# Penguin77jp/RaytracingMin

Hardware: AMD Instinct MI355X
Metric: Msamples/s (W*H*spp/s), Cornell box 1080p@1024spp (higher is better)
Workload: dtype f64; 1 GPU; cornellBoxSetting.json rows 0:1080 of 1920x1080 1024spp (SS 4 x S 64), L1 repaired, max_bounces 8, seed 0x5EED, host-libm sin/cos (RTM_MODE_HOST_TRIG), interleaved 8-row bands over 1 GPU(s) + one gather; sample_split_waves_per_tile=8, collective=none (one rank, frame stays in HBM)

## Files before the change

### raytracingmin_amd/csrc/rtm_kernels.hip

```cpp
#include <hip/hip_runtime.h>

#include <cfloat>
#include <cmath>
#include <cstdio>
#include <cstdlib>
#include <cstring>
#include <algorithm>
#include <atomic>
#include <thread>
#include <map>
#include <memory>
#include <mutex>
#include <shared_mutex>
#include <tuple>
#include <string>
#include <type_traits>
#include <vector>

#include "../../include/rtm.h"
#include "rtm_device.h"
#include "rtm_host.h"
#include "rtm_path.h"
#include "rtm_scene_facts.h"

// ... 709 lines not shown
    }
    return false;
}

template <class M, int UNROLL, typename RecT, int WPE, unsigned F>
static void launch_render_depth(const RenderParams& P, unsigned grid, hipStream_t stream) {
    const size_t pad = debug_lds_pad();
    if constexpr ((F & kPack8) != 0 && sizeof(RecT) == 1) {
        if (P.max_bounces >= 0 && P.max_bounces <= 8 && P.scene.n < 256) {
            if constexpr ((F & kDefer) != 0 && UNROLL == -8) {
                if (launch_exact_n<M, F, RecT, 16, WPE>(P, grid, stream)) return;
            }
            launch_tiles<M, F, UNROLL, RecT, 16, WPE>(P, grid, pad, stream);
            return;
        }
    }
    if constexpr ((F & kDefer) != 0 && sizeof(RecT) == 1) {
        if (P.scene.n < 256) {
            constexpr unsigned FL = (F & ~(kPack8 | kSteal)) | kPackL;
            if constexpr (UNROLL == -8) {
                if (launch_exact_n<M, FL, RecT, 0, WPE>(P, grid, stream)) return;
            }
            launch_tiles<M, FL, UNROLL, RecT, 0, WPE>(P, grid, pad, stream);
            return;
        }
    }
    constexpr unsigned FR = F & (kLdsTab | kPark | kStamp);
    if (!needs_pool(P)) launch_tiles<M, FR, UNROLL, RecT, 16, WPE>(P, grid, pad, stream);
    else launch_tiles<M, FR, UNROLL, RecT, deep_lds_levels<RecT>(), WPE>(P, grid, pad, stream);
}

template <int UNROLL, unsigned F>
static void launch_fold(const RenderParams& P, unsigned grid, hipStream_t stream) {
    if (P.split > 1) {
        launch_render_depth<MathFast, UNROLL, uint8_t, 4, F | kSplit>(P, P.split_first + P.n_tiles * P.split, stream);
        launch_split_finalize(P, stream);
    } else {
        launch_render_depth<MathFast, UNROLL, uint8_t, 4, F>(P, grid, stream);
    }
    if constexpr ((F & kSteal) != 0) launch_steal_finalize(P, grid, stream);
}
template <unsigned F>
static void launch_fold_lds(const RenderParams& P, unsigned grid, hipStream_t stream) {
    if (P.scene.n < 8) launch_fold<-8, F>(P, grid, stream);
    else launch_fold<8, F>(P, grid, stream);
}

static void launch_render(int variant, const RenderParams& P, unsigned grid, hipStream_t stream) {
    const int n = P.scene.n;
    constexpr unsigned kFold = kPark | kPack8 | kDefer;
    if (variant == kVariantFastLds && n > kLdsTableMaxSpheres) variant = kVariantFastGlobal;
    switch (variant) {
        case kVariantRef:
            if (n <= 256) launch_render_depth<MathRef, 1, uint8_t, 1, 0>(P, grid, stream);
            else launch_render_depth<MathRef, 1, uint32_t, 1, 0>(P, grid, stream);
            return;
        case kVariantFastLds:
            if (P.scene.plane != nullptr) launch_fold<8, kLdsTab | kFold | kPlanes>(P, grid, stream);
            else if (P.steal_ws != nullptr) launch_fold_lds<kLdsTab | kFold | kSteal>(P, grid, stream);
            else launch_fold_lds<kLdsTab | kFold>(P, grid, stream);
            return;
        case kVariantGlobalDefer:
            launch_fold<8, kFold>(P, grid, stream);
            return;
        case kVariantFp32: {
            const size_t lds = (((size_t)n * kFp32Row * sizeof(float) + 15) & ~(size_t)15) + 10 * sizeof(double);
            render_fp32_kernel<<<grid, 64, lds, stream>>>(P);
            return;
        }
        case kVariantPrimaryReuse:
            if (n < 8) launch_tiles<MathFast, kLdsTab | kFold | kReuse, -8, uint8_t, 16, 4>(P, grid, debug_lds_pad(), stream);
            else launch_tiles<MathFast, kLdsTab | kFold | kReuse, 8, uint8_t, 16, 4>(P, grid, debug_lds_pad(), stream);
            return;
// ... 1544 lines not shown
```

### raytracingmin_amd/csrc/rtm_kernels_tol.hip

```cpp
#define RTM_NS rtm_tol
#define RTM_TOL 1
#include <hip/hip_runtime.h>

#include <cmath>
#include <cstdlib>
#include <cstring>
#include <map>
#include <mutex>
#include <vector>

#include "rtm_internal.h"
#include "rtm_render_kernel.h"

namespace rtm_tol {

static bool compact_launch(const RenderParams& P) {
    const double cam = std::sqrt(P.cam_org.x * P.cam_org.x + P.cam_org.y * P.cam_org.y + P.cam_org.z * P.cam_org.z);
    return (P.scene.fold_flags & kSceneCompact) != 0u && cam <= kCompactExtent;
}
static bool expanded_form_launch(const RenderParams& P) {
    const unsigned e = (P.scene.fold_flags >> kSceneAxisReachShift) & kSceneAxisReachMask;
    const double cam = std::sqrt(P.cam_org.x * P.cam_org.x + P.cam_org.y * P.cam_org.y + P.cam_org.z * P.cam_org.z);
    return e != 0u && cam <= std::ldexp(1.0, (int)e - 128);
}
// ... 14 lines not shown
#define RTM_AXIS_CASE(k, sig)                                                                                    \
    if (P.scene.n == k && P.scene.axis_pat == ((sig) & 0xFFFFu) && ((shared_k << kAxisSharedKShift) | pairs) == ((sig) & ~0xFFFFu) && axis) { \
        launch_tiles<MathFast, F, axis_unroll(k, sig), uint8_t, LDS_D, kTolWavesPerSimd>(P, grid, lds_pad, stream); \
        return;                                                                                                  \
    }
    if constexpr (kPairsShape) {
        RTM_AXIS_CASE(7, kAxisSigCornell7Pairs)
    }
    RTM_AXIS_CASE(7, kAxisSigCornell7Walls)
#undef RTM_AXIS_CASE
#define RTM_AXIS_CASE(k, sig)                                                                                    \
    if (P.scene.n == k && P.scene.axis_pat == sig && axis) {                                                     \
        launch_tiles<MathFast, F, axis_unroll(k, sig), uint8_t, LDS_D, kTolWavesPerSimd>(P, grid, lds_pad, stream); \
        return;                                                                                                  \
    }
    if constexpr ((F & kPackL) != 0) {
        RTM_AXIS_CASE(7, kAxisSigCornell7)
    } else {
        RTM_AXIS_SIGNATURES(RTM_AXIS_CASE)
        switch (P.scene.n) {
            case 3: launch_tiles<MathFast, F, -103, uint8_t, LDS_D, kTolWavesPerSimd>(P, grid, lds_pad, stream); return;
            case 5: launch_tiles<MathFast, F, -105, uint8_t, LDS_D, kTolWavesPerSimd>(P, grid, lds_pad, stream); return;
            case 7: launch_tiles<MathFast, F, -107, uint8_t, LDS_D, kTolWavesPerSimd>(P, grid, lds_pad, stream); return;
            default: break;
        }
    }
#undef RTM_AXIS_CASE
    if (P.scene.n < 8) launch_tiles<MathFast, F, -8, uint8_t, LDS_D, kTolWavesPerSimd>(P, grid, lds_pad, stream);
    else launch_tiles<MathFast, F, 8, uint8_t, LDS_D, kTolWavesPerSimd>(P, grid, lds_pad, stream);
}

template <unsigned F>
static void launch_row(const RenderParams& P, unsigned grid, size_t lds_pad, hipStream_t stream) {
    if (P.split > 1) {
        launch_n<F | kSplit>(P, P.split_first + P.n_tiles * P.split, lds_pad, stream);
        launch_split_finalize(P, stream);
    } else {
        launch_n<F>(P, grid, lds_pad, stream);
    }
    if constexpr ((F & kSteal) != 0) launch_steal_finalize(P, grid, stream);
}

__global__ void tol_math_probe_kernel(int op, const double* __restrict__ a, const double* __restrict__ b, size_t n,
                                      double* __restrict__ out, const double2* __restrict__ tab) {
    const size_t i = (size_t)blockIdx.x * blockDim.x + threadIdx.x;
    if (i >= n) return;
    if (op >= 52 && op <= 54) {
        const size_t j = i & ~(size_t)7;
        double bb = 0.0, D4 = 0.0;
        if (b && j + 7 < n) {
            const D3 org = d3(a[j], a[j + 1], a[j + 2]), dir = d3(a[j + 3], a[j + 4], a[j + 5]);
            const unsigned pat = (unsigned)b[j];
            const double c = b[j + 1];
            if (pat >= 1u && pat <= 3u) {
                if (op == 52) {
                    const double4 g = double4{pat == 1u ? c : 0.0, pat == 2u ? c : 0.0, pat == 3u ? c : 0.0, b[j + 2]};
                    sphere_disc_ref(g, pat, org, dir, AxisSharedRef(org, dir), bb, D4);
                } else {
                    const AxisShared A(org, dir);
                    sphere_disc(double4{}, AxisRow{c, b[j + 3], b[j + 4]}, pat, op == 54, A.oo + b[j + 4], org, dir, A, bb, D4);
                }
            }
        }
        out[i] = (i & 7) == 0 ? bb : (i & 7) == 1 ? D4 : 0.0;
        return;
    }
    if (op == 55 || op == 56 || op == 61 || op == 62) {
        const size_t j = i & ~(size_t)7;
        double dis = DBL_MAX;
        int hit = -1;
        bool fell_back = false, general = false, again = false;
        if (b && n >= 56 && j + 7 < n) {
            const D3 org = d3(a[j], a[j + 1], a[j + 2]), dir = d3(a[j + 3], a[j + 4], a[j + 5]);
            SceneGlobal sc{};
            sc.v.geom = reinterpret_cast<const double4*>(b);
            sc.v.n = 7;
            if (op == 55) sphere_chunk<MathFast, 7, SceneGlobal, false, kAxisSigCornell7Pairs>(sc, 0, org, dir, dis, hit, &fell_back);
            else if (op == 61) sphere_chunk<MathFast, 7, SceneGlobal, false, kAxisSigCornell7Pairs>(sc, 0, org, dir, dis, hit, &fell_back, &general, &again);
            else if (op == 62) sphere_chunk<MathFast, 7, SceneGlobal, false, kAxisSigCornell7Pairs, true>(sc, 0, org, dir, dis, hit, &fell_back, &general, &again);
            else sphere_chunk<MathFast, 7, SceneGlobal, false, kAxisSigCornell7Walls>(sc, 0, org, dir, dis, hit);
        }
        const bool f2 = op >= 61 ? general : fell_back, f3 = op >= 61 && fell_back;
        const unsigned s = (unsigned)(i & 7);
        out[i] = s == 0u ? dis : s == 1u ? (double)hit : s == 2u ? (f2 ? 1.0 : 0.0) : s == 3u ? (f3 ? 1.0 : 0.0) : s == 4u ? (again ? 1.0 : 0.0) : 0.0;
        return;
    }
    if (op == 57 || op == 58) {
        if (i * 8 + 7 >= n) return;
        const double* q = a + i * 8;
        const RngPixelKey pk{(uint32_t)q[0], (uint32_t)q[1]};
        RngStream st{(uint32_t)q[2], (uint32_t)q[3]};
        const uint32_t n_next = (uint32_t)q[4];
        const bool ended = q[5] != 0.0;
        uint32_t w[4] = {0u, 0u, 0u, 0u};
        (void)rng_next_mi(st);
        if (op == 57) {
            const RngStream m = rng_merged_mix(ended, pk, n_next, st);
            if (ended) {
                w[2] = m.ctr;
                w[3] = m.k1;
            } else {
                w[0] = rng_bits_to_mi(m.ctr);
                w[1] = (uint32_t)(rng_bits_to_u01(m.k1) * 16777216.0);
                w[2] = st.ctr + 2u * 0x9E3779B9u;
                w[3] = st.k1;
            }
        } else if (ended) {
            st = rng_open(pk, n_next);
            w[2] = st.ctr;
            w[3] = st.k1;
        } else {
            w[0] = rng_next_mi(st);
            w[1] = (uint32_t)(rng_next(st) * 16777216.0);
            w[2] = st.ctr;
            w[3] = st.k1;
        }
// ... 183 lines not shown
```

### raytracingmin_amd/csrc/rtm_render_kernel.h

```cpp
#pragma once
#include <type_traits>

#include "rtm_path.h"

namespace RTM_NS {

struct RenderParams {
    SceneView scene;
    int W, H, S, SS;
    int row_begin, row_end;
    int band_count, band_index;
    int tiles_x;
    int mode, max_bounces;
    unsigned total_samples;
    unsigned sample_begin, sample_end, seeded;
    double preview_scale;
    float rate;
    double dSS, dS;
    double inv_ss, inv_s;
    D3 cam_org, ax, by, cz;
    uint64_t seed_mult;
    double* __restrict__ out64;
    float* __restrict__ out32;
    uint8_t* __restrict__ out8;
// ... 1014 lines not shown
        }
    }

    if constexpr (PARK) acc = d3(park[0 * 64 + lane], park[1 * 64 + lane], park[2 * 64 + lane]);
    if (STEAL && whole) {
    } else if (whole) {
        int px, py;
        pixel_xy(px, py);
        store_pixel(P, (px < P.W) && (py < P.row_end), px, py, acc);
    } else if (n_first == P.sample_begin) {
        unsigned hf, split_tile;
        split_wave(hf, split_tile);
        double* dst = P.partial + (size_t)split_tile * 192 + lane;
        dst[0] = acc.x;
        dst[64] = acc.y;
        dst[128] = acc.z;
    }
    if (P.counters) {
        if constexpr (DEFER) {
            if (lane == 0) {
                atomicAdd(P.counters + 0, (unsigned long long)w_casts);
                atomicAdd(P.counters + 1, (unsigned long long)w_bounces);
                atomicAdd(P.counters + 2, (unsigned long long)w_draws);
            }
        } else {
            wave_add_counter(P.counters + 0, pc.casts);
            wave_add_counter(P.counters + 1, pc.bounces);
            wave_add_counter(P.counters + 2, pc.draws);
        }
        if (stack.overflow) atomicOr(P.counters + 3, 1ull);
    }
}

__global__ __launch_bounds__(256) void split_finalize_kernel(const RenderParams P) {
    extern __shared__ __attribute__((aligned(16))) unsigned char lds_raw[];
    double* slot = reinterpret_cast<double*>(lds_raw);
    unsigned* present = reinterpret_cast<unsigned*>(slot + (size_t)P.split_len * 64u * 3u);
    const int tid = threadIdx.x, lane = tid & 63, chan = tid >> 6;
    const unsigned tile = frame_tile(P, P.split_first + blockIdx.x);
    if (tile == ~0u) return;
    const int tx = tile % P.tiles_x, ty = tile / P.tiles_x;
    const int px = tx * 8 + (lane & 7), py = band_row(P, ty, lane >> 3);
    const bool valid = (px < P.W) && (py < P.row_end);
    const unsigned plane_sz = P.split_len * 64u;
    double acc = chan < 3 ? P.partial[(size_t)blockIdx.x * 192 + chan * 64 + lane] : 0.0;
    for (unsigned f = 1; f < P.split; ++f) {
        const unsigned char* rows = P.contrib + ((size_t)blockIdx.x * (P.split - 1u) + (f - 1u)) * P.split_len * kTermRowBytes;
        unsigned n_terms = P.split_counts[(size_t)blockIdx.x * (P.split - 1u) + (f - 1u)];
        n_terms = n_terms <= plane_sz ? n_terms : 0u;
        for (unsigned m = (unsigned)tid; m < P.split_len * 2u; m += 256u) present[m] = 0u;
        __syncthreads();
        for (unsigned e = (unsigned)tid; e < n_terms; e += 256u) {
            const unsigned char* row = rows + (size_t)(e >> 6) * kTermRowBytes;
            const double* v = reinterpret_cast<const double*>(row) + (e & 63u);
            const unsigned tag = reinterpret_cast<const unsigned short*>(row + 3 * 64 * sizeof(double))[e & 63u];
            if ((tag >> 6) >= P.split_len) continue;
            const unsigned at = (tag >> 6) * 64u + (tag & 63u);
            slot[at] = v[0];
            slot[plane_sz + at] = v[64];
            slot[2 * plane_sz + at] = v[128];
            atomicOr(&present[(tag >> 6) * 2u + ((tag >> 5) & 1u)], 1u << (tag & 31u));
        }
        __syncthreads();
        if (chan < 3) {
            const double* mine = slot + (size_t)chan * plane_sz + lane;
            const unsigned* bits = present + (lane >> 5);
            for (unsigned m = 0; m < P.split_len; ++m)
                if ((bits[m * 2u] >> (lane & 31)) & 1u) acc = acc + mine[m * 64u];
        }
        __syncthreads();
    }
    if (chan < 3) slot[chan * 64 + lane] = acc;
    __syncthreads();
    if (chan == 0) store_pixel(P, valid, px, py, d3(slot[lane], slot[64 + lane], slot[128 + lane]));
}

__global__ __launch_bounds__(64) void steal_finalize_kernel(const RenderParams P) {
    extern __shared__ __attribute__((aligned(16))) unsigned char lds_raw[];
    unsigned short* idx = reinterpret_cast<unsigned short*>(lds_raw);
    const int lane = threadIdx.x;
    const unsigned tile = blockIdx.x;
    const unsigned ftile = frame_tile(P, tile);
    if (ftile == ~0u) return;
    const int tx = ftile % P.tiles_x, ty = ftile / P.tiles_x;
    const int px = tx * 8 + (lane & 7), py = band_row(P, ty, lane >> 3);
    const bool valid = (px < P.W) && (py < P.row_end);
    const unsigned char* blk = P.steal_ws + (size_t)tile * steal_tile_bytes(P.steal_rows);
    unsigned n_terms = reinterpret_cast<const unsigned*>(blk)[0];
    unsigned end_own = reinterpret_cast<const unsigned short*>(blk + 128)[lane];
    n_terms = n_terms <= P.steal_rows * 64u ? n_terms : 0u;
    const unsigned floor_chk = P.sample_end > P.steal_depth ? P.sample_end - P.steal_depth : 0u;
    end_own = (n_terms != 0u && end_own >= floor_chk && end_own <= P.sample_end) ? end_own : P.sample_end;
    const double* part = reinterpret_cast<const double*>(blk + kStealHdrBytes) + lane;
    D3 acc = d3(part[0], part[64], part[128]);
    if (n_terms != 0u) {
        const unsigned total = P.sample_end;
        const unsigned floor_s = total > P.steal_depth ? total - P.steal_depth : 0u;
        const unsigned char* rows = blk + kStealHdrBytes + 3 * 64 * sizeof(double);
        for (unsigned k = (unsigned)lane; k < P.steal_depth * 32u; k += 64u) reinterpret_cast<unsigned*>(idx)[k] = 0xFFFFFFFFu;
        __syncthreads();
        for (unsigned e = (unsigned)lane; e < n_terms; e += 64u) {
            const unsigned tag = reinterpret_cast<const unsigned*>(rows + (size_t)(e >> 6) * kStealRowBytes + 3 * 64 * sizeof(double))[e & 63u];
            const unsigned ts = tag & 0xFFFFu, tv = (tag >> 16) & 63u;
            if (ts >= floor_s && ts < total) idx[(ts - floor_s) * 64u + tv] = (unsigned short)e;
        }
        __syncthreads();
        if (valid) {
            for (unsigned s = end_own; s < total; ++s) {
                const unsigned e = idx[(s - floor_s) * 64u + (unsigned)lane];
                if (e >= n_terms) continue;
                const double* v = reinterpret_cast<const double*>(rows + (size_t)(e >> 6) * kStealRowBytes) + (e & 63u);
                acc = acc + d3(v[0], v[64], v[128]);
            }
        }
    }
    store_pixel(P, valid, px, py, acc);
}

template <class M, unsigned F, int UNROLL, typename RecT, int LDS_D, int WPE>
void launch_tiles(RenderParams P, unsigned grid, size_t pad, hipStream_t stream) {
    const size_t lds = render_lds_bytes<F, RecT, LDS_D>(P.scene.n, lds_rows_for(UNROLL), pad, &P.unit_tab);
    render_tiles_kernel<M, F, UNROLL, RecT, LDS_D, WPE><<<grid, 64, lds, stream>>>(P);
}
inline void launch_split_finalize(const RenderParams& P, hipStream_t stream) {
    split_finalize_kernel<<<P.n_tiles, 256, (size_t)P.split_len * (64 * 3 * sizeof(double) + 2 * sizeof(unsigned)), stream>>>(P);
}
inline void launch_steal_finalize(const RenderParams& P, unsigned grid, hipStream_t stream) {
    const unsigned n_whole = P.split > 1 ? P.split_first : grid;
    if (n_whole) steal_finalize_kernel<<<n_whole, 64, (size_t)P.steal_depth * 64 * sizeof(unsigned short), stream>>>(P);
}

__global__ __launch_bounds__(64) void prim_prepass_kernel(const RenderParams P, unsigned long long* __restrict__ masks,
                                                          double* __restrict__ dirs) {
    const int lane = threadIdx.x;
    const unsigned tile = blockIdx.x;
    const unsigned ftile = frame_tile(P, tile);
    if (ftile == ~0u) return;
    auto store_dir = [&](const unsigned sub, const D3 d) {
        const unsigned all_s = (unsigned)(P.SS * P.SS);
        double* q = dirs + ((size_t)tile * all_s + sub) * 192 + (unsigned)lane;
        constexpr int kStep = 64;
        __builtin_nontemporal_store(d.x, q);
        __builtin_nontemporal_store(d.y, q + kStep);
        __builtin_nontemporal_store(d.z, q + 2 * kStep);
    };
    const int x = (int)(ftile % (unsigned)P.tiles_x) * 8 + (lane & 7);
    const int y = band_row(P, (int)(ftile / (unsigned)P.tiles_x), lane >> 3);
    const double cam[9] = {P.ax.x, P.ax.y, P.ax.z, P.by.x, P.by.y, P.by.z, P.cz.x, P.cz.y, P.cz.z};
    [[maybe_unused]] unsigned long long mask = 0ull;
    const unsigned all = (unsigned)(P.SS * P.SS);
    const unsigned sub_end = (P.sample_end - 1u) / (unsigned)P.S + 2u;
    for (unsigned sub = P.sample_begin / (unsigned)P.S; sub < (sub_end < all ? sub_end : all); ++sub) {
        if (dirs == nullptr && (masks == nullptr || sub >= 64u)) break;
        const D3 d = primary_dir_lds(P, cam, x, y, (int)(sub / (unsigned)P.SS) + 1, (int)(sub % (unsigned)P.SS) + 1);
#if RTM_TOL
        if (masks != nullptr && sub < 64u) {
            SceneGlobal sc;
            sc.v = P.scene;
            mask |= primary_tie_risk(sc, P.cam_org, d) ? (1ull << sub) : 0ull;
        }
#endif
        if (dirs != nullptr) store_dir(sub, d);
// ... 8 lines not shown
```

### raytracingmin_amd/csrc/rtm_path.h

```cpp
#pragma once
#include <cfloat>
#include <type_traits>

#include "../../include/rtm.h"
#include "rtm_device.h"
#include "rtm_grid_header.h"
#include "rtm_scene_flags.h"

namespace RTM_NS {


__device__ __forceinline__ double seq_rcp(const double y) {
    double r = __builtin_amdgcn_rcp(y);
    double e = __builtin_fma(-y, r, 1.0);
#if RTM_TOL
    return __builtin_fma(r, __builtin_fma(e, e, e), r);
#else
    r = __builtin_fma(r, e, r);
    e = __builtin_fma(-y, r, 1.0);
    return __builtin_fma(r, e, r);
#endif
}
__device__ __forceinline__ double seq_quot(const double x, const double y, const double r) {
#if RTM_TOL
    (void)y;
    return x * r;
#else
    const double q = x * r;
    const double rem = __builtin_fma(-y, q, x);
    return __builtin_fma(rem, r, q);
#endif
}
#if RTM_TOL
__device__ __forceinline__ double half_of_rsq(const double y) {
    return __hiloint2double(__double2hiint(y) - 0x00100000, __double2loint(y));
// ... 704 lines not shown
            t1v[k] = __hiloint2double((int)sel_u32_mask(le, 0x7FF80000u, (uint32_t)__double2hiint(t1)), (int)lo);
        } else {
            const double t2 = b[k] + sq[k];
            const unsigned long long near = __builtin_amdgcn_ballot_w64(t1 > 0.001);
            far |= __builtin_amdgcn_ballot_w64(t2 >= (double)1e-5f) & ~near;
            t1v[k] = __hiloint2double((int)sel_u32_mask(near, (uint32_t)__double2hiint(t1), 0x7FF80000u), (int)lo);
        }
    }
    if (WALLS != 0u && far != 0ull) {
        if (asked_again) *asked_again = true;
        far = 0ull;
#pragma unroll
        for (int k = 0; k < K; ++k) {
            const double t1 = b[k] - sq[k], t2 = b[k] + sq[k];
            far |= __builtin_amdgcn_ballot_w64(t2 >= (double)1e-5f) & ~__builtin_amdgcn_ballot_w64(t1 > 0.001);
        }
    }
    if (far == 0ull) {
        double best = dis;
#pragma unroll
        for (int k = 0; k < K; ++k) {
            double m;
            asm("v_min_f64 %0, %1, %2" : "=v"(m) : "v"(best), "v"(t1v[k]));
            best = m;
        }
        dis = best;
        hit_object = (int)((((uint32_t)__double2loint(best)) + 1u) & 7u) - 1;
        return;
    }
#endif
    if (general) *general = true;
#pragma unroll
    for (int k = 0; k < K; ++k) accept_update(b[k], sq[k], (int)idx[k], dis, hit_object);
}

#if RTM_TOL
struct AxisRow {
    double c, m2c, K;
};
__device__ __forceinline__ AxisRow load_axis_row_uniform(const double4* geom, int i) {
#if defined(__HIP_DEVICE_COMPILE__)
    typedef const __attribute__((address_space(4))) double* ConstF64Ptr;
    ConstF64Ptr p = (ConstF64Ptr)(unsigned long long)(geom + i);
    return AxisRow{p[0], p[1], p[2]};
#else
    return AxisRow{geom[i].x, geom[i].y, geom[i].z};
#endif
}
struct AxisShared {
    double od, oo;
    __device__ __forceinline__ AxisShared(const D3 org, const D3 dir) : od(dot(org, dir)), oo(dot(org, org)) {}
};
struct AxisSharedRef {
    double Pyz, Pxz, Pxy, Qyz, Qxz, Qxy;
    __device__ __forceinline__ AxisSharedRef(const D3 org, const D3 dir) {
        const double px = org.x * dir.x, py = org.y * dir.y, pz = org.z * dir.z;
        const double qx = org.x * org.x, qy = org.y * org.y, qz = org.z * org.z;
        Pyz = py + pz; Pxz = px + pz; Pxy = px + py;
        Qyz = qy + qz; Qxz = qx + qz; Qxy = qx + qy;
    }
};
#else
struct AxisShared {
    double Px, Py, Pz, Pxy, Qx, Qy, Qz, Qxy;
    __device__ __forceinline__ AxisShared(const D3 org, const D3 dir) {
        const double px = org.x * dir.x, py = org.y * dir.y, pz = org.z * dir.z;
// ... 42 lines not shown
        D4 = b * b - (py * py + A.Qxz) + g.w;
    } else if (pat == 3u) {
        const double pz = g.z - org.z;
        b = pz * dir.z - A.Pxy;
        D4 = b * b - (A.Qxy + pz * pz) + g.w;
    } else {
        const D3 p_o = d3(g.x - org.x, g.y - org.y, g.z - org.z);
        b = dot(p_o, dir);
        D4 = b * b - dot(p_o, p_o) + g.w;
    }
}
__device__ __forceinline__ double pair_signed_origin(const unsigned pat, const D3 org, const D3 dir) {
    const double oa = pat == 1u ? org.x : pat == 2u ? org.y : org.z;
    const double da = pat == 1u ? dir.x : pat == 2u ? dir.y : dir.z;
#if defined(__HIP_DEVICE_COMPILE__)
    const uint32_t hi = __builtin_amdgcn_bitop3_b32((uint32_t)__double2hiint(oa), (uint32_t)__double2hiint(da), 0x80000000u, 0x78);
#else
    const uint32_t hi = (uint32_t)__double2hiint(oa) ^ ((uint32_t)__double2hiint(da) & 0x80000000u);
#endif
    return __hiloint2double((int)hi, __double2loint(oa));
}
__device__ __forceinline__ bool pair_unproven(const AxisRow r, const unsigned pat, const double ooK, const D3 org, const D3 dir,
                                              const AxisShared& A) {
    const double da = pat == 1u ? dir.x : pat == 2u ? dir.y : dir.z;
    double bu;
#if defined(__HIP_DEVICE_COMPILE__)
    asm("v_fma_f64 %0, -%1, |%2|, -%3" : "=v"(bu) : "s"(r.c), "v"(da), "v"(A.od));
#else
    bu = __builtin_fma(-r.c, __builtin_fabs(da), -A.od);
#endif
    const double qu = __builtin_fma(-r.m2c, pair_signed_origin(pat, org, dir), ooK);
    return !(bu <= -kPairBeta && __builtin_fma(-2.0 * kPairTau, bu, qu) >= 0.0);
}
__device__ __forceinline__ void pair_disc(const AxisRow r, const unsigned pat, const double ooK, const D3 org, const D3 dir,
                                          const AxisShared& A, double& b, double& D4) {
    const double da = pat == 1u ? dir.x : pat == 2u ? dir.y : dir.z;
#if defined(__HIP_DEVICE_COMPILE__)
    asm("v_fma_f64 %0, %1, |%2|, -%3" : "=v"(b) : "s"(r.c), "v"(da), "v"(A.od));
#else
    b = __builtin_fma(r.c, __builtin_fabs(da), -A.od);
#endif
    D4 = __builtin_fma(b, b, -__builtin_fma(r.m2c, pair_signed_origin(pat, org, dir), ooK));
}
__device__ __forceinline__ uint32_t pair_index(const unsigned pat, const D3 dir, const int lower) {
    const double da = pat == 1u ? dir.x : pat == 2u ? dir.y : dir.z;
    return (uint32_t)lower + ((uint32_t)__double2hiint(da) >> 31);
}
#else
__device__ __forceinline__ void sphere_disc(const double4 g, const unsigned pat, const D3 org, const D3 dir,
                                            const AxisShared& A, double& b, double& D4) {
    if (pat == 1u) {
        const double px = g.x - org.x;
        b = px * dir.x - A.Py - A.Pz;
        D4 = b * b - (px * px + A.Qy + A.Qz) + g.w;
    } else if (pat == 2u) {
        const double py = g.y - org.y;
        b = py * dir.y - A.Px - A.Pz;
        D4 = b * b - (A.Qx + py * py + A.Qz) + g.w;
    } else if (pat == 3u) {
        const double pz = g.z - org.z;
        b = pz * dir.z - A.Pxy;
        D4 = b * b - (A.Qxy + pz * pz) + g.w;
    } else {
        const D3 p_o = d3(g.x - org.x, g.y - org.y, g.z - org.z);
        b = dot(p_o, dir);
        D4 = b * b - dot(p_o, p_o) + g.w;
    }
}
#endif

template <class M, int K, bool EARLY_OUT = false>
__device__ __forceinline__ void sphere_chunk_g(const double4 (&g)[K], const int i0, const D3 org, const D3 dir,
                                               double& dis, int& hit_object) {
    double b[K], D4[K], sq[K];
#pragma unroll
    for (int k = 0; k < K; ++k) {
        const D3 p_o = d3(g[k].x - org.x, g[k].y - org.y, g[k].z - org.z);
        b[k] = dot(p_o, dir);
        D4[k] = b[k] * b[k] - dot(p_o, p_o) + g[k].w;
    }
    if constexpr (EARLY_OUT) {
        double top = D4[0];
#pragma unroll
        for (int k = 1; k < K; ++k) top = __builtin_fmax(top, D4[k]);
        if (__builtin_amdgcn_ballot_w64(top >= 0.0) == 0) return;
#pragma unroll
        for (int k = 0; k < K; ++k) {
            if (__builtin_amdgcn_ballot_w64(D4[k] >= 0.0) == 0) continue;
            const double sqk = M::sqrt64(D4[k]);
            const double t1 = b[k] - sqk, t2 = b[k] + sqk;
            const double t = (t1 > 0.001) ? t1 : t2;
            const bool accept = (t < dis) && !(t < (double)1e-5f);
            dis = accept ? t : dis;
            hit_object = accept ? i0 + k : hit_object;
        }
        return;
    }
    M::template sqrt64_batch_hit<K>(D4, sq);
#pragma unroll
    for (int k = 0; k < K; ++k) accept_update(b[k], sq[k], i0 + k, dis, hit_object);
}
constexpr int kGeomPhase = 2;
constexpr unsigned pair_wall_slots(const int K, const unsigned KMP) {
    unsigned slots = 0u;
    for (int k = 0; k < K; ++k) {
        const int rank = __builtin_popcount(KMP & ((1u << k) - 1u));
        if (((KMP >> k) & 1u) != 0u && (rank & 1) == 0) slots |= 1u << (k - rank / 2);
    }
    return slots;
}
static_assert(pair_wall_slots(7, 0x7Eu) == 0xEu, "the Cornell box: the lamp in slot 0, a wall pair in each of slots 1 to 3");
template <class M, int K, class Scene, bool EARLY_OUT = false, unsigned SIG = 0u, bool ACCEPT_T2 = false>
__device__ __forceinline__ void sphere_chunk(const Scene& sc, const int i0, const D3 org, const D3 dir,
                                             double& dis, int& hit_object, bool* pairs_fell_back = nullptr,
                                             bool* accept_general = nullptr, bool* accept_again = nullptr) {
    static_assert(SIG == 0u || (K > kGeomPhase && K < 8 && !EARLY_OUT), "an axis signature names the spheres of ONE exact chunk");
    constexpr int PH = kGeomPhase;
    if constexpr (K > PH && !EARLY_OUT) {
        double b[K], D4[K], sq[K];
        if constexpr (SIG != 0u) {
            const AxisShared A(org, dir);
#if RTM_TOL
            if constexpr ((SIG & kAxisPairsBit) != 0u) {
                constexpr unsigned KMP = (SIG >> kAxisSharedKShift) & 0xFFu;
                constexpr int KC = K - __builtin_popcount(KMP) / 2;
                double pooK = 0.0;
                bool unproven = false;
#pragma unroll
                for (int k = 0; k < K; ++k) {
                    const int rank = __builtin_popcount(KMP & ((1u << k) - 1u));
                    if (((KMP >> k) & 1u) == 0u || (rank & 1) != 0) continue;
                    const AxisRow r = load_axis_row_uniform(sc.v.geom, K + i0 + k);
                    if (rank == 0) pooK = A.oo + r.K;
                    unproven |= pair_unproven(r, (SIG >> (2 * k)) & 3u, pooK, org, dir, A);
                }
                if (__builtin_amdgcn_ballot_w64(unproven) == 0ull) {
                    double pb[KC], pD4[KC], psq[KC];
                    uint32_t idx[KC];
#pragma unroll
                    for (int k = 0; k < K; ++k) {
                        const unsigned pat = (SIG >> (2 * k)) & 3u;
                        const int rank = __builtin_popcount(KMP & ((1u << k) - 1u));
                        const bool member = ((KMP >> k) & 1u) != 0u;
                        if (member && (rank & 1) != 0) continue;
                        const int slot = k - rank / 2;
                        if (member) pair_disc(load_axis_row_uniform(sc.v.geom, K + i0 + k), pat, pooK, org, dir, A, pb[slot], pD4[slot]);
                        else if (pat != 0u) sphere_disc(double4{}, load_axis_row_uniform(sc.v.geom, K + i0 + k), pat, false, 0.0, org, dir, A, pb[slot], pD4[slot]);
                        else sphere_disc(sc.geom_uniform(i0 + k), AxisRow{}, 0u, false, 0.0, org, dir, A, pb[slot], pD4[slot]);
                    }
                    M::template sqrt64_batch_hit<KC, true>(pD4, psq);
#pragma unroll
                    for (int k = 0; k < K; ++k) {
                        const int rank = __builtin_popcount(KMP & ((1u << k) - 1u));
                        const bool member = ((KMP >> k) & 1u) != 0u;
                        if (member && (rank & 1) != 0) continue;
                        idx[k - rank / 2] = member ? pair_index((SIG >> (2 * k)) & 3u, dir, i0 + k) : (uint32_t)(i0 + k);
                    }
                    accept_batch_lane<KC, ACCEPT_T2 ? 0u : pair_wall_slots(K, KMP)>(pb, psq, idx, dis, hit_object, accept_general,
                                                                                   accept_again);
                    return;
                }
                if (pairs_fell_back) *pairs_fell_back = true;
            }
            double ooK = 0.0;
#endif
            constexpr int PA = 2;
#pragma unroll
            for (int k0 = 0; k0 < K; k0 += PA) {
#if RTM_TOL
                constexpr unsigned KM = (SIG >> kAxisSharedKShift) & 0xFFu;
                double4 g[PA] = {};
                AxisRow r[PA] = {};
#pragma unroll
                for (int k = 0; k < PA; ++k)
                    if (k0 + k < K) {
                        if (((SIG >> (2 * (k0 + k))) & 3u) != 0u) r[k] = load_axis_row_uniform(sc.v.geom, K + i0 + k0 + k);
                        else g[k] = sc.geom_uniform(i0 + k0 + k);
                    }
#pragma unroll
                for (int k = 0; k < PA; ++k)
                    if (k0 + k < K) {
                        const bool shared_k = ((KM >> (k0 + k)) & 1u) != 0u;
                        if (shared_k && (KM & ((1u << (k0 + k)) - 1u)) == 0u) ooK = A.oo + r[k].K;
                        sphere_disc(g[k], r[k], (SIG >> (2 * (k0 + k))) & 3u, shared_k, ooK, org, dir, A, b[k0 + k], D4[k0 + k]);
                    }
#else
                double4 g[PA];
#pragma unroll
                for (int k = 0; k < PA; ++k)
                    if (k0 + k < K) g[k] = sc.geom_uniform(i0 + k0 + k);
#pragma unroll
                for (int k = 0; k < PA; ++k)
                    if (k0 + k < K) sphere_disc(g[k], (SIG >> (2 * (k0 + k))) & 3u, org, dir, A, b[k0 + k], D4[k0 + k]);
// ... 342 lines not shown
template <class M, int UNROLL, class Scene>
__device__ __forceinline__ int nearest_hit(const Scene& sc, const D3 org, const D3 dir, double& dis) {
    int hit_object = -1;
    dis = DBL_MAX;
    const int n = sc.n();
    if constexpr (UNROLL == 0 || UNROLL == 1) {
        for (int i = 0; i < n; ++i) {
            const double4 g = sc.geom_uniform(i);
            double t;
            bool hit;
            if (sc.v.plane != nullptr && g.w < 0.0)
                hit = plane_test(sc.v.plane + (size_t)i * 16, org, dir, t);
            else
                hit = sphere_test<M>(g, org, dir, t);
            if (hit && t < dis && t > 0) {
                dis = t;
                hit_object = i;
            }
        }
    } else {
        if constexpr (Scene::kPlanes) {
            int i0 = 0;
            for (; i0 + 4 <= n; i0 += 4) object_chunk<M, 4>(sc, i0, org, dir, dis, hit_object);
            switch (n - i0) {
                case 1: object_chunk<M, 1>(sc, i0, org, dir, dis, hit_object); break;
                case 2: object_chunk<M, 2>(sc, i0, org, dir, dis, hit_object); break;
                case 3: object_chunk<M, 3>(sc, i0, org, dir, dis, hit_object); break;
                default: break;
            }
            return hit_object;
        }
        if constexpr (UNROLL <= -1000) {
            constexpr int code = -UNROLL - 1000;
            sphere_chunk<M, (code & 7), Scene, false, (unsigned)(code >> 3)>(sc, 0, org, dir, dis, hit_object);
            return hit_object;
        }
        if constexpr (UNROLL <= -101 && UNROLL >= -107) {
            sphere_chunk<M, -UNROLL - 100>(sc, 0, org, dir, dis, hit_object);
            return hit_object;
        }
        constexpr int U = UNROLL <= -101 ? 8 : (UNROLL < 0 ? -UNROLL : UNROLL);
        static_assert(U == 8 || U == 4, "chunks of 8 or 4 plus an exact tail");
        int i0 = 0;
        if constexpr (UNROLL > 0) {
            for (; i0 + U <= n; i0 += U) sphere_chunk<M, U>(sc, i0, org, dir, dis, hit_object);
        }
        switch (n - i0) {
            case 1: sphere_chunk<M, 1>(sc, i0, org, dir, dis, hit_object); break;
            case 2: sphere_chunk<M, 2>(sc, i0, org, dir, dis, hit_object); break;
            case 3: sphere_chunk<M, 3>(sc, i0, org, dir, dis, hit_object); break;
            case 4: sphere_chunk<M, 4>(sc, i0, org, dir, dis, hit_object); break;
            case 5: sphere_chunk<M, 5>(sc, i0, org, dir, dis, hit_object); break;
            case 6: sphere_chunk<M, 6>(sc, i0, org, dir, dis, hit_object); break;
            case 7: sphere_chunk<M, 7>(sc, i0, org, dir, dis, hit_object); break;
            default: break;
        }
    }
    return hit_object;
}

#if RTM_TOL
template <class Scene>
__device__ __forceinline__ int nearest_hit_exactfp(const Scene& sc, const D3 org, const D3 dir, double& dis) {
#pragma clang fp contract(off)
    int hit_object = -1;
    dis = DBL_MAX;
    const int n = sc.n();
// ... 534 lines not shown
```

Baseline: 26830 Msamples/s.

## Merge split and steal finalize kernels into one windowed ordered-accumulation launch

```diff
diff --git a/raytracingmin_amd/csrc/rtm_kernels.hip b/raytracingmin_amd/csrc/rtm_kernels.hip
--- a/raytracingmin_amd/csrc/rtm_kernels.hip
+++ b/raytracingmin_amd/csrc/rtm_kernels.hip
@@ -765,13 +765,9 @@
 
 template <int UNROLL, unsigned F>
 static void launch_fold(const RenderParams& P, unsigned grid, hipStream_t stream) {
-    if (P.split > 1) {
-        launch_render_depth<MathFast, UNROLL, uint8_t, 4, F | kSplit>(P, P.split_first + P.n_tiles * P.split, stream);
-        launch_split_finalize(P, stream);
-    } else {
-        launch_render_depth<MathFast, UNROLL, uint8_t, 4, F>(P, grid, stream);
-    }
-    if constexpr ((F & kSteal) != 0) launch_steal_finalize(P, grid, stream);
+    if (P.split > 1) launch_render_depth<MathFast, UNROLL, uint8_t, 4, F | kSplit>(P, P.split_first + P.n_tiles * P.split, stream);
+    else launch_render_depth<MathFast, UNROLL, uint8_t, 4, F>(P, grid, stream);
+    launch_finalize(P, grid, (F & kSteal) != 0, stream);
 }
 template <unsigned F>
 static void launch_fold_lds(const RenderParams& P, unsigned grid, hipStream_t stream) {
diff --git a/raytracingmin_amd/csrc/rtm_kernels_tol.hip b/raytracingmin_amd/csrc/rtm_kernels_tol.hip
--- a/raytracingmin_amd/csrc/rtm_kernels_tol.hip
+++ b/raytracingmin_amd/csrc/rtm_kernels_tol.hip
@@ -70,13 +70,9 @@
 
 template <unsigned F>
 static void launch_row(const RenderParams& P, unsigned grid, size_t lds_pad, hipStream_t stream) {
-    if (P.split > 1) {
-        launch_n<F | kSplit>(P, P.split_first + P.n_tiles * P.split, lds_pad, stream);
-        launch_split_finalize(P, stream);
-    } else {
-        launch_n<F>(P, grid, lds_pad, stream);
-    }
-    if constexpr ((F & kSteal) != 0) launch_steal_finalize(P, grid, stream);
+    if (P.split > 1) launch_n<F | kSplit>(P, P.split_first + P.n_tiles * P.split, lds_pad, stream);
+    else launch_n<F>(P, grid, lds_pad, stream);
+    launch_finalize(P, grid, (F & kSteal) != 0, stream);
 }
 
 __global__ void tol_math_probe_kernel(int op, const double* __restrict__ a, const double* __restrict__ b, size_t n,
diff --git a/raytracingmin_amd/csrc/rtm_render_kernel.h b/raytracingmin_amd/csrc/rtm_render_kernel.h
--- a/raytracingmin_amd/csrc/rtm_render_kernel.h
+++ b/raytracingmin_amd/csrc/rtm_render_kernel.h
@@ -1070,102 +1070,131 @@
     }
 }
 
-__global__ __launch_bounds__(256) void split_finalize_kernel(const RenderParams P) {
-    extern __shared__ __attribute__((aligned(16))) unsigned char lds_raw[];
-    double* slot = reinterpret_cast<double*>(lds_raw);
-    unsigned* present = reinterpret_cast<unsigned*>(slot + (size_t)P.split_len * 64u * 3u);
-    const int tid = threadIdx.x, lane = tid & 63, chan = tid >> 6;
-    const unsigned tile = frame_tile(P, P.split_first + blockIdx.x);
-    if (tile == ~0u) return;
-    const int tx = tile % P.tiles_x, ty = tile / P.tiles_x;
-    const int px = tx * 8 + (lane & 7), py = band_row(P, ty, lane >> 3);
-    const bool valid = (px < P.W) && (py < P.row_end);
-    const unsigned plane_sz = P.split_len * 64u;
-    double acc = chan < 3 ? P.partial[(size_t)blockIdx.x * 192 + chan * 64 + lane] : 0.0;
-    for (unsigned f = 1; f < P.split; ++f) {
-        const unsigned char* rows = P.contrib + ((size_t)blockIdx.x * (P.split - 1u) + (f - 1u)) * P.split_len * kTermRowBytes;
-        unsigned n_terms = P.split_counts[(size_t)blockIdx.x * (P.split - 1u) + (f - 1u)];
-        n_terms = n_terms <= plane_sz ? n_terms : 0u;
-        for (unsigned m = (unsigned)tid; m < P.split_len * 2u; m += 256u) present[m] = 0u;
+constexpr unsigned kFinalizeWindow = 64;
+constexpr unsigned kFinalizeChunk = 8;
+template <bool TAG32, bool PRE0>
+__device__ __forceinline__ void add_terms_in_order(D3& acc, unsigned short* idx, unsigned win, const unsigned char* rows,
+                                                   unsigned n_terms, unsigned lo, unsigned hi, unsigned from, unsigned pre0) {
+    constexpr size_t ROW_BYTES = TAG32 ? kStealRowBytes : kTermRowBytes;
+    constexpr size_t TAG_AT = 3 * 64 * sizeof(double);
+    const unsigned lane = threadIdx.x;
+    for (unsigned w = lo; w < hi; w += win) {
+        const unsigned n = hi - w < win ? hi - w : win;
+        const unsigned n_up = (n + kFinalizeChunk - 1u) / kFinalizeChunk * kFinalizeChunk;
+        for (unsigned k = lane; k < n_up * 8u; k += 64u) reinterpret_cast<uint4*>(idx)[k] = make_uint4(~0u, ~0u, ~0u, ~0u);
         __syncthreads();
-        for (unsigned e = (unsigned)tid; e < n_terms; e += 256u) {
-            const unsigned char* row = rows + (size_t)(e >> 6) * kTermRowBytes;
-            const double* v = reinterpret_cast<const double*>(row) + (e & 63u);
-            const unsigned tag = reinterpret_cast<const unsigned short*>(row + 3 * 64 * sizeof(double))[e & 63u];
-            if ((tag >> 6) >= P.split_len) continue;
-            const unsigned at = (tag >> 6) * 64u + (tag & 63u);
-            slot[at] = v[0];
-            slot[plane_sz + at] = v[64];
-            slot[2 * plane_sz + at] = v[128];
-            atomicOr(&present[(tag >> 6) * 2u + ((tag >> 5) & 1u)], 1u << (tag & 31u));
+        for (unsigned e0 = 0; e0 < n_terms; e0 += 256u) {
+            unsigned tag[4];
+#pragma unroll
+            for (unsigned j = 0; j < 4u; ++j) {
+                const unsigned e = e0 + j * 64u + lane;
+                tag[j] = 0u;
+                if (PRE0 && e0 == 0u && j == 0u) {
+                    tag[j] = pre0;
+                } else if (e < n_terms) {
+                    const unsigned char* t = rows + (size_t)(e >> 6) * ROW_BYTES + TAG_AT;
+                    tag[j] = TAG32 ? reinterpret_cast<const unsigned*>(t)[e & 63u] : (unsigned)reinterpret_cast<const unsigned short*>(t)[e & 63u];
+                }
+            }
+#pragma unroll
+            for (unsigned j = 0; j < 4u; ++j) {
+                const unsigned e = e0 + j * 64u + lane;
+                const unsigned ts = TAG32 ? (tag[j] & 0xFFFFu) : (tag[j] >> 6), tv = TAG32 ? ((tag[j] >> 16) & 63u) : (tag[j] & 63u);
+                if (e < n_terms && ts - w < n) idx[(ts - w) * 64u + tv] = (unsigned short)e;
+            }
         }
         __syncthreads();
-        if (chan < 3) {
-            const double* mine = slot + (size_t)chan * plane_sz + lane;
-            const unsigned* bits = present + (lane >> 5);
-            for (unsigned m = 0; m < P.split_len; ++m)
-                if ((bits[m * 2u] >> (lane & 31)) & 1u) acc = acc + mine[m * 64u];
+        for (unsigned c = 0; c < n; c += kFinalizeChunk) {
+            unsigned at[kFinalizeChunk];
+            bool some = false;
+#pragma unroll
+            for (unsigned j = 0; j < kFinalizeChunk; ++j) {
+                at[j] = idx[(c + j) * 64u + lane];
+                at[j] = (at[j] < n_terms && w + c + j >= from) ? at[j] : 0xFFFFFFFFu;
+                some = some || at[j] != 0xFFFFFFFFu;
+            }
+            if (!__any(some)) continue;
+            double vx[kFinalizeChunk], vy[kFinalizeChunk], vz[kFinalizeChunk];
+#pragma unroll
+            for (unsigned j = 0; j < kFinalizeChunk; ++j) {
+                vx[j] = vy[j] = vz[j] = 0.0;
+                if (at[j] != 0xFFFFFFFFu) {
+                    const double* v = reinterpret_cast<const double*>(rows + (size_t)(at[j] >> 6) * ROW_BYTES) + (at[j] & 63u);
+                    vx[j] = v[0];
+                    vy[j] = v[64];
+                    vz[j] = v[128];
+                }
+            }
+#pragma unroll
+            for (unsigned j = 0; j < kFinalizeChunk; ++j)
+                if (at[j] != 0xFFFFFFFFu) acc = acc + d3(vx[j], vy[j], vz[j]);
         }
         __syncthreads();
     }
-    if (chan < 3) slot[chan * 64 + lane] = acc;
-    __syncthreads();
-    if (chan == 0) store_pixel(P, valid, px, py, d3(slot[lane], slot[64 + lane], slot[128 + lane]));
-}
-
-__global__ __launch_bounds__(64) void steal_finalize_kernel(const RenderParams P) {
+}
+
+__global__ __launch_bounds__(64) void finalize_kernel(const RenderParams P, const unsigned n_steal, const unsigned win) {
     extern __shared__ __attribute__((aligned(16))) unsigned char lds_raw[];
     unsigned short* idx = reinterpret_cast<unsigned short*>(lds_raw);
     const int lane = threadIdx.x;
-    const unsigned tile = blockIdx.x;
+    const bool steal_role = blockIdx.x < n_steal;
+    const unsigned tile = steal_role ? blockIdx.x : P.split_first + (blockIdx.x - n_steal);
     const unsigned ftile = frame_tile(P, tile);
     if (ftile == ~0u) return;
     const int tx = ftile % P.tiles_x, ty = ftile / P.tiles_x;
     const int px = tx * 8 + (lane & 7), py = band_row(P, ty, lane >> 3);
     const bool valid = (px < P.W) && (py < P.row_end);
-    const unsigned char* blk = P.steal_ws + (size_t)tile * steal_tile_bytes(P.steal_rows);
-    unsigned n_terms = reinterpret_cast<const unsigned*>(blk)[0];
-    unsigned end_own = reinterpret_cast<const unsigned short*>(blk + 128)[lane];
-    n_terms = n_terms <= P.steal_rows * 64u ? n_terms : 0u;
-    const unsigned floor_chk = P.sample_end > P.steal_depth ? P.sample_end - P.steal_depth : 0u;
-    end_own = (n_terms != 0u && end_own >= floor_chk && end_own <= P.sample_end) ? end_own : P.sample_end;
-    const double* part = reinterpret_cast<const double*>(blk + kStealHdrBytes) + lane;
-    D3 acc = d3(part[0], part[64], part[128]);
-    if (n_terms != 0u) {
+    D3 acc;
+    if (steal_role) {
+        const unsigned char* blk = P.steal_ws + (size_t)tile * steal_tile_bytes(P.steal_rows);
+        const unsigned char* rows = blk + kStealHdrBytes + 3 * 64 * sizeof(double);
+        unsigned n_terms = reinterpret_cast<const unsigned*>(blk)[0];
+        unsigned end_own = reinterpret_cast<const unsigned short*>(blk + 128)[lane];
+        const double* part = reinterpret_cast<const double*>(blk + kStealHdrBytes) + lane;
+        acc = d3(part[0], part[64], part[128]);
+        const unsigned pre0 = P.steal_rows != 0u ? reinterpret_cast<const unsigned*>(rows + 3 * 64 * sizeof(double))[lane] : 0u;
+        n_terms = n_terms <= P.steal_rows * 64u ? n_terms : 0u;
         const unsigned total = P.sample_end;
         const unsigned floor_s = total > P.steal_depth ? total - P.steal_depth : 0u;
-        const unsigned char* rows = blk + kStealHdrBytes + 3 * 64 * sizeof(double);
-        for (unsigned k = (unsigned)lane; k < P.steal_depth * 32u; k += 64u) reinterpret_cast<unsigned*>(idx)[k] = 0xFFFFFFFFu;
-        __syncthreads();
-        for (unsigned e = (unsigned)lane; e < n_terms; e += 64u) {
-            const unsigned tag = reinterpret_cast<const unsigned*>(rows + (size_t)(e >> 6) * kStealRowBytes + 3 * 64 * sizeof(double))[e & 63u];
-            const unsigned ts = tag & 0xFFFFu, tv = (tag >> 16) & 63u;
-            if (ts >= floor_s && ts < total) idx[(ts - floor_s) * 64u + tv] = (unsigned short)e;
-        }
-        __syncthreads();
-        if (valid) {
-            for (unsigned s = end_own; s < total; ++s) {
-                const unsigned e = idx[(s - floor_s) * 64u + (unsigned)lane];
-                if (e >= n_terms) continue;
-                const double* v = reinterpret_cast<const double*>(rows + (size_t)(e >> 6) * kStealRowBytes) + (e & 63u);
-                acc = acc + d3(v[0], v[64], v[128]);
-            }
+        end_own = (n_terms != 0u && end_own >= floor_s && end_own <= total) ? end_own : total;
+        if (n_terms != 0u) {
+            unsigned lo = end_own;
+            for (int off = 32; off > 0; off >>= 1) {
+                const unsigned o = (unsigned)__shfl_xor((int)lo, off, 64);
+                lo = o < lo ? o : lo;
+            }
+            add_terms_in_order<true, true>(acc, idx, win, rows, n_terms, lo, total, valid ? end_own : total, pre0);
+        }
+    } else {
+        const unsigned st = blockIdx.x - n_steal;
+        const double* part = P.partial + (size_t)st * 192 + lane;
+        acc = d3(part[0], part[64], part[128]);
+        for (unsigned f = 1; f < P.split; ++f) {
+            const size_t wave = (size_t)st * (P.split - 1u) + (f - 1u);
+            unsigned n_terms = P.split_counts[wave];
+            n_terms = n_terms <= P.split_len * 64u ? n_terms : 0u;
+            if (n_terms != 0u)
+                add_terms_in_order<false, false>(acc, idx, win, P.contrib + wave * P.split_len * kTermRowBytes, n_terms, 0u, P.split_len, 0u, 0u);
         }
     }
     store_pixel(P, valid, px, py, acc);
 }
+
 
 template <class M, unsigned F, int UNROLL, typename RecT, int LDS_D, int WPE>
 void launch_tiles(RenderParams P, unsigned grid, size_t pad, hipStream_t stream) {
     const size_t lds = render_lds_bytes<F, RecT, LDS_D>(P.scene.n, lds_rows_for(UNROLL), pad, &P.unit_tab);
     render_tiles_kernel<M, F, UNROLL, RecT, LDS_D, WPE><<<grid, 64, lds, stream>>>(P);
 }
-inline void launch_split_finalize(const RenderParams& P, hipStream_t stream) {
-    split_finalize_kernel<<<P.n_tiles, 256, (size_t)P.split_len * (64 * 3 * sizeof(double) + 2 * sizeof(unsigned)), stream>>>(P);
-}
-inline void launch_steal_finalize(const RenderParams& P, unsigned grid, hipStream_t stream) {
-    const unsigned n_whole = P.split > 1 ? P.split_first : grid;
-    if (n_whole) steal_finalize_kernel<<<n_whole, 64, (size_t)P.steal_depth * 64 * sizeof(unsigned short), stream>>>(P);
+inline void launch_finalize(const RenderParams& P, unsigned grid, bool steal, hipStream_t stream) {
+    const unsigned n_split = P.split > 1 ? P.n_tiles : 0u;
+    const unsigned n_steal = !steal ? 0u : P.split > 1 ? P.split_first : grid;
+    if (n_steal + n_split == 0u) return;
+    unsigned win = n_steal ? P.steal_depth : 0u;
+    if (n_split && P.split_len > win) win = P.split_len;
+    win = win < 1u ? 1u : (win > kFinalizeWindow ? kFinalizeWindow : win);
+    const unsigned lds_rows = (win + kFinalizeChunk - 1u) / kFinalizeChunk * kFinalizeChunk;
+    finalize_kernel<<<n_steal + n_split, 64, (size_t)lds_rows * 64 * sizeof(unsigned short), stream>>>(P, n_steal, win);
 }
 
 __global__ __launch_bounds__(64) void prim_prepass_kernel(const RenderParams P, unsigned long long* __restrict__ masks,
```

Result: no change. 27060 Msamples/s (median of 6 runs) (+0.9%).

## Rescue single-unproven wall pair by testing its far wall before general fallback

Applied to the files above, without the earlier changes.

```diff
diff --git a/raytracingmin_amd/csrc/rtm_kernels_tol.hip b/raytracingmin_amd/csrc/rtm_kernels_tol.hip
--- a/raytracingmin_amd/csrc/rtm_kernels_tol.hip
+++ b/raytracingmin_amd/csrc/rtm_kernels_tol.hip
@@ -103,11 +103,12 @@
         out[i] = (i & 7) == 0 ? bb : (i & 7) == 1 ? D4 : 0.0;
         return;
     }
-    if (op == 55 || op == 56 || op == 61 || op == 62) {
+    if (op == 55 || op == 56 || op == 61 || op == 62 || op == 63) {
         const size_t j = i & ~(size_t)7;
         double dis = DBL_MAX;
         int hit = -1;
         bool fell_back = false, general = false, again = false;
+        int route = 0;
         if (b && n >= 56 && j + 7 < n) {
             const D3 org = d3(a[j], a[j + 1], a[j + 2]), dir = d3(a[j + 3], a[j + 4], a[j + 5]);
             SceneGlobal sc{};
@@ -116,10 +117,15 @@
             if (op == 55) sphere_chunk<MathFast, 7, SceneGlobal, false, kAxisSigCornell7Pairs>(sc, 0, org, dir, dis, hit, &fell_back);
             else if (op == 61) sphere_chunk<MathFast, 7, SceneGlobal, false, kAxisSigCornell7Pairs>(sc, 0, org, dir, dis, hit, &fell_back, &general, &again);
             else if (op == 62) sphere_chunk<MathFast, 7, SceneGlobal, false, kAxisSigCornell7Pairs, true>(sc, 0, org, dir, dis, hit, &fell_back, &general, &again);
+            else if (op == 63) sphere_chunk<MathFast, 7, SceneGlobal, false, kAxisSigCornell7Pairs, false, true>(sc, 0, org, dir, dis, hit, &fell_back, &general, &again, &route);
             else sphere_chunk<MathFast, 7, SceneGlobal, false, kAxisSigCornell7Walls>(sc, 0, org, dir, dis, hit);
         }
         const bool f2 = op >= 61 ? general : fell_back, f3 = op >= 61 && fell_back;
         const unsigned s = (unsigned)(i & 7);
+        if (op == 63) {
+            out[i] = s == 0u ? dis : s == 1u ? (double)hit : s == 2u ? (fell_back ? 4.0 : (double)route) : s == 3u ? (general ? 1.0 : 0.0) : s == 4u ? (again ? 1.0 : 0.0) : 0.0;
+            return;
+        }
         out[i] = s == 0u ? dis : s == 1u ? (double)hit : s == 2u ? (f2 ? 1.0 : 0.0) : s == 3u ? (f3 ? 1.0 : 0.0) : s == 4u ? (again ? 1.0 : 0.0) : 0.0;
         return;
     }
diff --git a/raytracingmin_amd/csrc/rtm_path.h b/raytracingmin_amd/csrc/rtm_path.h
--- a/raytracingmin_amd/csrc/rtm_path.h
+++ b/raytracingmin_amd/csrc/rtm_path.h
@@ -1,6 +1,5 @@
 #pragma once
 #include <cfloat>
-#include <type_traits>
 
 #include "../../include/rtm.h"
 #include "rtm_device.h"
@@ -771,6 +770,21 @@
     if (general) *general = true;
 #pragma unroll
     for (int k = 0; k < K; ++k) accept_update(b[k], sq[k], (int)idx[k], dis, hit_object);
+}
+__device__ __forceinline__ bool accept_one_more(const double b, const double sq, const uint32_t idx, double& dis) {
+#if defined(__HIP_DEVICE_COMPILE__)
+    const double t1 = b - sq, t2 = b + sq;
+    const unsigned long long near = __builtin_amdgcn_ballot_w64(t1 > 0.001);
+    if ((__builtin_amdgcn_ballot_w64(t2 >= (double)1e-5f) & ~near) != 0ull) return false;
+    const uint32_t lo = ((uint32_t)__double2loint(t1) & ~7u) | idx;
+    const double t1v = __hiloint2double(t1 > 0.001 ? __double2hiint(t1) : (int)0x7FF80000u, (int)lo);
+    double m;
+    asm("v_min_f64 %0, %1, %2" : "=v"(m) : "v"(dis), "v"(t1v));
+    dis = m;
+    return true;
+#else
+    return false;
+#endif
 }
 
 #if RTM_TOL
@@ -879,6 +893,18 @@
     const double qu = __builtin_fma(-r.m2c, pair_signed_origin(pat, org, dir), ooK);
     return !(bu <= -kPairBeta && __builtin_fma(-2.0 * kPairTau, bu, qu) >= 0.0);
 }
+__device__ __forceinline__ unsigned long long pair_unproven_mask(const AxisRow r, const unsigned pat, const double ooK, const D3 org,
+                                                                 const D3 dir, const AxisShared& A) {
+#if defined(__HIP_DEVICE_COMPILE__)
+    const double da = pat == 1u ? dir.x : pat == 2u ? dir.y : dir.z;
+    double bu;
+    asm("v_fma_f64 %0, -%1, |%2|, -%3" : "=v"(bu) : "s"(r.c), "v"(da), "v"(A.od));
+    const double qu = __builtin_fma(-r.m2c, pair_signed_origin(pat, org, dir), ooK);
+    return __builtin_amdgcn_ballot_w64(!(bu <= -kPairBeta)) | __builtin_amdgcn_ballot_w64(!(__builtin_fma(-2.0 * kPairTau, bu, qu) >= 0.0));
+#else
+    return pair_unproven(r, pat, ooK, org, dir, A) ? 1ull : 0ull;
+#endif
+}
 __device__ __forceinline__ void pair_disc(const AxisRow r, const unsigned pat, const double ooK, const D3 org, const D3 dir,
                                           const AxisShared& A, double& b, double& D4) {
     const double da = pat == 1u ? dir.x : pat == 2u ? dir.y : dir.z;
@@ -892,6 +918,20 @@
 __device__ __forceinline__ uint32_t pair_index(const unsigned pat, const D3 dir, const int lower) {
     const double da = pat == 1u ? dir.x : pat == 2u ? dir.y : dir.z;
     return (uint32_t)lower + ((uint32_t)__double2hiint(da) >> 31);
+}
+__device__ __forceinline__ void pair_other_disc(const AxisRow r, const unsigned pat, const double ooK, const D3 org, const D3 dir,
+                                                const AxisShared& A, double& b, double& D4) {
+    const double da = pat == 1u ? dir.x : pat == 2u ? dir.y : dir.z;
+#if defined(__HIP_DEVICE_COMPILE__)
+    asm("v_fma_f64 %0, -%1, |%2|, -%3" : "=v"(b) : "s"(r.c), "v"(da), "v"(A.od));
+#else
+    b = __builtin_fma(-r.c, __builtin_fabs(da), -A.od);
+#endif
+    D4 = __builtin_fma(b, b, -__builtin_fma(-r.m2c, pair_signed_origin(pat, org, dir), ooK));
+}
+__device__ __forceinline__ uint32_t pair_other_index(const unsigned pat, const D3 dir, const int lower) {
+    const double da = pat == 1u ? dir.x : pat == 2u ? dir.y : dir.z;
+    return (uint32_t)lower + 1u - ((uint32_t)__double2hiint(da) >> 31);
 }
 #else
 __device__ __forceinline__ void sphere_disc(const double4 g, const unsigned pat, const D3 org, const D3 dir,
@@ -957,10 +997,11 @@
     return slots;
 }
 static_assert(pair_wall_slots(7, 0x7Eu) == 0xEu, "the Cornell box: the lamp in slot 0, a wall pair in each of slots 1 to 3");
-template <class M, int K, class Scene, bool EARLY_OUT = false, unsigned SIG = 0u, bool ACCEPT_T2 = false>
+template <class M, int K, class Scene, bool EARLY_OUT = false, unsigned SIG = 0u, bool ACCEPT_T2 = false, bool PAIR_EXTRA = false>
 __device__ __forceinline__ void sphere_chunk(const Scene& sc, const int i0, const D3 org, const D3 dir,
                                              double& dis, int& hit_object, bool* pairs_fell_back = nullptr,
-                                             bool* accept_general = nullptr, bool* accept_again = nullptr) {
+                                             bool* accept_general = nullptr, bool* accept_again = nullptr,
+                                             int* pair_route = nullptr) {
     static_assert(SIG == 0u || (K > kGeomPhase && K < 8 && !EARLY_OUT), "an axis signature names the spheres of ONE exact chunk");
     constexpr int PH = kGeomPhase;
     if constexpr (K > PH && !EARLY_OUT) {
@@ -971,19 +1012,54 @@
             if constexpr ((SIG & kAxisPairsBit) != 0u) {
                 constexpr unsigned KMP = (SIG >> kAxisSharedKShift) & 0xFFu;
                 constexpr int KC = K - __builtin_popcount(KMP) / 2;
+                static_assert(!(PAIR_EXTRA && ACCEPT_T2), "the probe's reference form keeps the wave-level fallback");
                 double pooK = 0.0;
-                bool unproven = false;
+                unsigned long long un_any = 0ull;
+                int flagged = 0, which = 0;
 #pragma unroll
                 for (int k = 0; k < K; ++k) {
                     const int rank = __builtin_popcount(KMP & ((1u << k) - 1u));
                     if (((KMP >> k) & 1u) == 0u || (rank & 1) != 0) continue;
                     const AxisRow r = load_axis_row_uniform(sc.v.geom, K + i0 + k);
                     if (rank == 0) pooK = A.oo + r.K;
-                    unproven |= pair_unproven(r, (SIG >> (2 * k)) & 3u, pooK, org, dir, A);
+                    const unsigned long long un = pair_unproven_mask(r, (SIG >> (2 * k)) & 3u, pooK, org, dir, A);
+                    un_any |= un;
+                    if constexpr (PAIR_EXTRA) {
+                        flagged += un != 0ull ? 1 : 0;
+                        which = un != 0ull ? 1 + rank / 2 : which;
+                    }
                 }
-                if (__builtin_amdgcn_ballot_w64(unproven) == 0ull) {
+                bool one_more = false;
+                if constexpr (PAIR_EXTRA) {
+                    if (__builtin_expect(un_any != 0ull, 0)) {
+                        const bool finite = __builtin_fabs(A.od) < __builtin_inf() && __builtin_fabs(pooK) < __builtin_inf();
+                        if (flagged == 1 && __builtin_amdgcn_ballot_w64(!finite) == 0ull) {
+                            AxisShared A2 = A;
+                            double pooK2 = pooK;
+#if defined(__HIP_DEVICE_COMPILE__)
+                            asm volatile("" : "+v"(A2.od), "+v"(pooK2));
+#endif
+                            double ob[1] = {0.0}, oD4[1] = {0.0}, osq[1];
+                            uint32_t oidx = 0u;
+#pragma unroll
+                            for (int k = 0; k < K; ++k) {
+                                const int rank = __builtin_popcount(KMP & ((1u << k) - 1u));
+                                if (((KMP >> k) & 1u) == 0u || (rank & 1) != 0 || which != 1 + rank / 2) continue;
+                                const unsigned pat = (SIG >> (2 * k)) & 3u;
+                                pair_other_disc(load_axis_row_uniform(sc.v.geom, K + i0 + k), pat, pooK2, org, dir, A2, ob[0], oD4[0]);
+                                oidx = pair_other_index(pat, dir, i0 + k);
+                            }
+                            if (__builtin_amdgcn_ballot_w64((unsigned)__double2hiint(oD4[0]) < 0x10000000u) == 0ull) {
+                                seq_sqrt_batch<1, true>(oD4, osq);
+                                one_more = accept_one_more(ob[0], osq[0], oidx, dis);
+                            }
+                        }
+                    }
+                }
+                if (un_any == 0ull || one_more) {
                     double pb[KC], pD4[KC], psq[KC];
                     uint32_t idx[KC];
+                    bool general = false;
 #pragma unroll
                     for (int k = 0; k < K; ++k) {
                         const unsigned pat = (SIG >> (2 * k)) & 3u;
@@ -1003,9 +1079,19 @@
                         if (member && (rank & 1) != 0) continue;
                         idx[k - rank / 2] = member ? pair_index((SIG >> (2 * k)) & 3u, dir, i0 + k) : (uint32_t)(i0 + k);
                     }
-                    accept_batch_lane<KC, ACCEPT_T2 ? 0u : pair_wall_slots(K, KMP)>(pb, psq, idx, dis, hit_object, accept_general,
-                                                                                   accept_again);
-                    return;
+                    accept_batch_lane<KC, ACCEPT_T2 ? 0u : pair_wall_slots(K, KMP)>(pb, psq, idx, dis, hit_object,
+                                                                                   PAIR_EXTRA ? &general : accept_general, accept_again);
+                    if (__builtin_expect(!PAIR_EXTRA || !one_more, 1)) {
+                        if (PAIR_EXTRA && accept_general && general) *accept_general = true;
+                        return;
+                    }
+                    if (!general) {
+                        if (pair_route) *pair_route = which;
+                        return;
+                    }
+                    dis = DBL_MAX;
+                    hit_object = -1;
+                    if (accept_again) *accept_again = false;
                 }
                 if (pairs_fell_back) *pairs_fell_back = true;
             }
@@ -1414,7 +1500,7 @@
         }
         if constexpr (UNROLL <= -1000) {
             constexpr int code = -UNROLL - 1000;
-            sphere_chunk<M, (code & 7), Scene, false, (unsigned)(code >> 3)>(sc, 0, org, dir, dis, hit_object);
+            sphere_chunk<M, (code & 7), Scene, false, (unsigned)(code >> 3), false, true>(sc, 0, org, dir, dis, hit_object);
             return hit_object;
         }
         if constexpr (UNROLL <= -101 && UNROLL >= -107) {
```

Result: slower. 26800 Msamples/s before, 26210 Msamples/s after (-2.2%).
